# immunogenomics/harmony

Hardware: AMD Instinct MI355X
Metric: cells_per_sec_to_convergence (higher is better)
Workload: dtype f32

## Files before the change

### harmony_amd/csrc/hmx_api_diag.inc

```
int hmx_debug_seq_oe(const float* R, int64_t n, int32_t K, const int32_t* level, int32_t B, const int32_t* list, int64_t nlist,
                     const int32_t* chain_off, const int32_t* chain_cnt, int32_t nchains, int32_t seg_cells, int32_t passes, float* totals,
                     int64_t* mismatch, double* residual) {
  if (!R || !list || !level || !chain_off || !chain_cnt || !totals || n <= 0 || K <= 0 || B <= 0 || nchains <= 0 || seg_cells <= 0 || passes < 2) return HMX_ERR_ARG;
  if (nlist <= 0 || n > 2000000000ll || nlist > 2000000000ll || (size_t)B * 256 > 60 * 1024) return HMX_ERR_ARG;
  for (int64_t i = 0; i < nlist; i++) if (list[i] < 0 || list[i] >= n) return HMX_ERR_ARG;
  for (int64_t i = 0; i < n; i++) if (level[i] < 0 || level[i] >= B) return HMX_ERR_ARG;
  for (int c = 0; c < nchains; c++) if (chain_off[c] < 0 || chain_cnt[c] < 0 || (int64_t)chain_off[c] + chain_cnt[c] > nlist) return HMX_ERR_ARG;
  hmx_ctx* ctx = hmx_create();
  float* dR = nullptr; int* dl = nullptr; int* dlev = nullptr; int* dq = nullptr;
  auto run = [&]() -> int {
    int ndev = 0;
    if (hipGetDeviceCount(&ndev) != hipSuccess || ndev <= 0) return fail(ctx, HMX_ERR_DEVICE, "no HIP device");
    HIPCHK(hipStreamCreateWithFlags(&ctx->L.stream, hipStreamNonBlocking)); ctx->own_stream = true;
    HIPCHK(hipMalloc((void**)&dR, sizeof(float) * (size_t)n * K)); HIPCHK(hipMalloc((void**)&dl, sizeof(int) * (size_t)nlist));
    HIPCHK(hipMalloc((void**)&dlev, sizeof(int) * (size_t)n)); HIPCHK(hipMalloc((void**)&dq, sizeof(int) * (size_t)B));
    std::vector<int> ident(B); std::iota(ident.begin(), ident.end(), 0);
    CHK(h2d(ctx, dR, R, (size_t)n * K)); CHK(h2d(ctx, dl, list, (size_t)nlist)); CHK(h2d(ctx, dlev, level, (size_t)n)); CHK(h2d(ctx, dq, ident.data(), (size_t)B));
    ctx->K = K; ctx->B = B; ctx->seq_passes = passes; ctx->seq_stats = true;
    ctx->D.R = dR; ctx->D.K = K; ctx->D.B = B; ctx->D.C = 1; ctx->D.combo = dlev; ctx->D.qlev = dq;
    for (int c = 0; c < 4; c++) ctx->D.cov_end[c] = B;
    std::vector<std::pair<int, int>> ch;
    for (int c = 0; c < nchains; c++) ch.push_back({chain_off[c], chain_cnt[c]});
    CHK(seq_plan_build(ctx, ctx->plan_round, ch, seg_cells));
    CHK(seq_run_oe(ctx, ctx->plan_round, dl, nullptr, 0, nchains));
// ... 128 lines not shown
    if (ctx->L.stream && hipStreamSynchronize(ctx->L.stream) != hipSuccess) return -1;
    if (ctx->side && hipStreamSynchronize(ctx->side) != hipSuccess) return -1;
    return scalar(1.0);
  }
  if (f == "chain") return scalar((ctx->chain_ok || ctx->D.chain_pair) ? 1.0 : 0.0);
  if (f == "chain_wgs") return scalar((double)ctx->chain_wgs);
  if (f == "chain_pair") return scalar(ctx->D.chain_pair ? 1.0 : 0.0);
  if (f == "dot_bf") return scalar(ctx->D.dot_bf ? 1.0 : 0.0);
  if (f == "sold_carry") return scalar(ctx->carry_ok ? 1.0 : 0.0);
  if (f == "carried_rounds") return scalar((double)ctx->carried_rounds);
  if (f == "rounds_without_R") return scalar((double)ctx->rounds_without_R);
  if (f == "chain_rounds") return scalar((double)ctx->chain_rounds);
  if (f == "shuffle_inv") return scalar(ctx->shuf_inv ? 1.0 : 0.0);
  if (f == "p2p:exchange_us") return scalar(ctx->p2p_exchange_us);
  if (f == "p2p:allreduce_calls") return scalar((double)ctx->p2p_ar_calls);
  if (f == "p2p:allreduce_big_windows") return scalar((double)ctx->p2p_ar_big_windows);
  if (f == "p2p") return scalar(ctx->p2p_on && ctx->p2p_world == ctx->world ? 1.0 : 0.0);
  if (f == "chain_dbg") {
    if (!ctx->ran_setup) return -1;
    if (!out) return 64;
    std::vector<unsigned long long> h(64);
    if (d2h(ctx, h.data(), ctx->D.chain_dbg, 64)) return -1;
    (void)hipMemsetAsync(ctx->D.chain_dbg, 0, sizeof(unsigned long long) * 64, ctx->L.stream);
    return vec(h);
  }
  if (f.rfind("gputimer:", 0) == 0) {
    resolve_phases(ctx);
    const std::string nm = f.substr(9);
    if (nm == "Rcells_update") return hmx_get(ctx, "prof:update_ms", out, cap);
    auto it = ctx->gpu_timers.find(nm); return scalar(it == ctx->gpu_timers.end() ? 0.0 : it->second);
  }
  if (f.rfind("timer:", 0) == 0) { auto it = ctx->timers.find(f.substr(6)); return scalar(it == ctx->timers.end() ? 0.0 : it->second); }
  if (f == "seed_cells") return vec(ctx->seed_cells);
  if (f == "Y") return vec(ctx->Y);
  if (f == "W") return vec(ctx->W);
  if (f == "Pr_b") return vec(ctx->Pr_b);
  if (f == "theta") return vec(ctx->theta);
  if (f == "sigma") return vec(ctx->sigma);
  if (f == "lambda") return vec(ctx->lambda);
  if (f == "B_vec") return vec(ctx->B_vec);
  if (f == "objective_kmeans") return vec(ctx->obj_kmeans);
  if (f == "objective_kmeans_dist") return vec(ctx->obj_dist);
  if (f == "objective_kmeans_entropy") return vec(ctx->obj_entropy);
  if (f == "objective_kmeans_cross") return vec(ctx->obj_cross);
  if (f == "objective_harmony") return vec(ctx->obj_harmony);
  if (f == "kmeans_rounds") return vec(ctx->kmeans_rounds);
  if (ctx->query_done && (f == "Z_corr" || f == "Z_orig" || f == "R")) return hmx_get_matrix(ctx, field, out, HMX_F64, HMX_HOST, cap);
  if (!ctx->ran_setup) return -1;
  if (hipSetDevice(ctx->device) != hipSuccess) return -1;
  if (f == "ref_Nr" || f == "ref_C") {
    if (ctx->ran_init && !ctx->R_valid) { ctx->err = "R is not available: the clustering call that would have stored it did not complete"; return -1; }
    if (sync_solve_results(ctx)) return -1;
    const int K = ctx->K, d = ctx->d;
    const int64_t cnt = f == "ref_Nr" ? K : (int64_t)K * d;
    if (!out) return cnt;
    std::vector<double> res;
    if (ref_summary(ctx, res)) return -1;
    std::vector<double> v((size_t)cnt);
    for (int k = 0; k < K; k++) {
      if (f == "ref_Nr") v[k] = res[(size_t)k * (d + 1) + d];
      else for (int j = 0; j < d; j++) v[k + (size_t)K * j] = res[(size_t)k * (d + 1) + j];
    }
    return vec(v);
  }
  if (f == "seq:mismatch" || f == "seq:residual") {
    if (!ctx->sq_mismatch) return scalar(0.0);
// ... 133 lines not shown
```

### harmony_amd/csrc/hmx_api_kmeans.inc

```
int gather_centres(hmx_ctx* ctx, const std::vector<long long>& gcells, long long* d_gcells, double* d_rows) {
  const int K = ctx->K, d = ctx->d;
  CHK(h2d(ctx, d_gcells, gcells.data(), (size_t)K));
  l_gather_rows(ctx->L, ctx->D, d_gcells, (uint64_t)ctx->goff, d_rows); KCHK();
  CHK(allreduce(ctx, d_rows, (int64_t)K * d, 1));
  l_y_images(ctx->L, ctx->D, d_rows, 0); KCHK();
  ctx->y_on_device = true;
  return 0;
}

int kmeans_centers(hmx_ctx* ctx) {
  const int K = ctx->K, d = ctx->d;
  const Dev& D = ctx->D;
  ctx->Y.assign((size_t)d * K, 0.f);
  long long* const d_gcells = D.km_gcells; double* const d_rows = D.km_rows; unsigned* const d_excl = D.km_excl;
  std::vector<long long> gcells(K);
  const float Nm1 = (float)((uint64_t)ctx->N_global - 1);
  const bool rmode = ctx->rng_mode == 1;
  if (rmode) ensure_rrng(ctx);
  for (int i = 0; i < K; i++) gcells[i] = (long long)std::floor((rmode ? ctx->rrng.arma_randu() : hmx_u01(ctx->seed, 0, (uint64_t)i)) * Nm1);
  CHK(gather_centres(ctx, gcells, d_gcells, d_rows));
  std::vector<unsigned long long> win(K), sentinel(K, SEED_SENTINEL);
  std::set<unsigned> sup;
  if (rmode) {
    const int64_t n = ctx->N;
// ... 37 lines not shown
  } else {
  CHK(h2d(ctx, D.seedmin, sentinel.data(), (size_t)K));
  auto seed_probe = [&](const unsigned* excl, int nexcl) -> int {
    ctx->D.seed_key = ctx->seed; ctx->D.seed_goff = (unsigned long long)ctx->goff; ctx->D.seed_excl = excl; ctx->D.seed_nexcl = nexcl;
    l_tile_static(ctx->L, ctx->D, 3); KCHK();
    return 0;
  };
  CHK(seed_probe(nullptr, 0));
  CHK(allreduce(ctx, D.seedmin, K, 2));
  CHK(d2h(ctx, win.data(), D.seedmin, (size_t)K));
  for (int i = 0; i < K; i++) {
    unsigned g = (unsigned)(win[i] & 0xffffffffu);
    if (win[i] == SEED_SENTINEL) return fail(ctx, HMX_ERR_STATE, "centroid seeding found no candidate cell");
    if (sup.count(g)) {
      std::vector<unsigned> ex(sup.begin(), sup.end());
      CHK(h2d(ctx, d_excl, ex.data(), ex.size()));
      CHK(h2d(ctx, D.seedmin, sentinel.data(), (size_t)K));
      CHK(seed_probe(d_excl, (int)ex.size()));
      CHK(allreduce(ctx, D.seedmin, K, 2));
      std::vector<unsigned long long> w2(K);
      CHK(d2h(ctx, w2.data(), D.seedmin, (size_t)K));
      if (w2[i] == SEED_SENTINEL) return fail(ctx, HMX_ERR_STATE, "centroid seeding ran out of distinct cells");
      g = (unsigned)(w2[i] & 0xffffffffu);
    }
    sup.insert(g);
    gcells[i] = (long long)g;
  }
  }
  ctx->seed_cells.assign(gcells.begin(), gcells.end());
  CHK(gather_centres(ctx, gcells, d_gcells, d_rows));
  const bool tile_ok = (size_t)D.NQ * D.NS * 1024 + ((size_t)K * d + K) * 8 <= 160 * 1024;
  for (int it = 0; it < 10; it++) {
    if (it == 0) HIPCHK(hipMemsetAsync(D.lsum, 0, sizeof(long long) * ((size_t)K * d + K), ctx->L.stream));
    if (tile_ok) { l_tile_static(ctx->L, D, 2); KCHK(); }
    else { l_lloyd(ctx->L, D); KCHK(); }
    CHK(allreduce(ctx, D.lsum, (int64_t)K * d + K, 0));
    l_lloyd_finish(ctx->L, D); KCHK();
  }
  ctx->y_on_device = true;
  return 0;
}

void apply_set(Dev& D, const hmx_ctx::SortSet& s) {
  D.blk = s.blk; D.lorder = s.lorder; D.lpair = s.lpair; D.lcombo = s.lcombo; D.boff = s.boff; D.binoff = s.binoff; D.counts = s.counts; D.offs = s.offs; D.blkv = s.blkv; D.bincnt = s.bincnt;
}
int sort_group(hmx_ctx* ctx, uint64_t first) {
  const int nr = 4 - (int)(first & 3);
  SortBatch Sb{};
  Dev Dt = ctx->D; Dt.nxt = ctx->carry_ok ? 1 : 0;
  if (ctx->shuf_inv) {
    ShufSets T{};
    for (int r = 0; r < nr; r++) {
      const int os = (int)((first + (uint64_t)r) & 3);
      const hmx_ctx::SortSet& t = ctx->sets[os];
      T.posr[r] = ctx->posr[os]; T.lpair[r] = t.lpair; T.lorder[r] = t.lorder; T.lcombo[r] = t.lcombo; T.boff[r] = t.boff; T.partcnt[r] = ctx->shuf_partcnt[os]; T.binbase[r] = t.binoff; T.bincnt[r] = t.bincnt; T.binacc[r] = ctx->shuf_binacc[os];
    }
    l_shuffle_inv(ctx->L, Dt, T, nr, ctx->seed, first, (uint64_t)ctx->N_global, (uint64_t)ctx->goff, ctx->cells_per_block); KCHK();
  } else {
  for (int r = 0; r < nr; r++) {
    const hmx_ctx::SortSet& t = ctx->sets[(first + (uint64_t)r) & 3];
    Sb.p[r] = SortPtrs{t.blk, t.blkv, t.counts, t.offs, t.binoff, t.bincnt, t.boff, t.lorder, t.lcombo, t.lpair};
  }
  l_sort_batch(ctx->L, Dt, Sb, nr, ctx->seed, first, (uint64_t)ctx->N_global, (uint64_t)ctx->goff, ctx->cells_per_block); KCHK();
  }
  for (int r = 0; r < nr; r++) {
    const int os = (int)((first + (uint64_t)r) & 3);
    ctx->sorted_round[os] = (int64_t)first + r; ctx->sorted_seed[os] = ctx->seed; ctx->sorted_nxt[os] = Dt.nxt != 0; ctx->sorted_on_side[os] = false;
  }
  return 0;
}
int prepare_round(hmx_ctx* ctx, uint64_t round) {
  Dev& D = ctx->D;
  const int sset = (int)(round & (uint64_t)ctx->oset_mask);
// ... 56 lines not shown
```

### harmony_amd/csrc/hmx_api_p2p.inc

```
int hmx_p2p_export(hmx_ctx* ctx, uint8_t* handle_out) {
  if (!ctx || !handle_out) return ctx ? fail(ctx, HMX_ERR_ARG, "null handle buffer") : HMX_ERR_ARG;
  static_assert(sizeof(hipIpcMemHandle_t) == HMX_P2P_HANDLE_BYTES, "HIP IPC handle size");
  if (ctx->device < 0) { int cur = 0; (void)hipGetDevice(&cur); ctx->device = cur; }
  HIPCHK(hipSetDevice(ctx->device));
  if (!ctx->p2p_self) {
    const char* m = getenv("HMX_P2P_MEM");
    const unsigned flags = (m && std::string(m) == "uncached") ? hipDeviceMallocUncached : hipDeviceMallocFinegrained;
    void* p = nullptr;
    HIPCHK(hipExtMallocWithFlags(&p, P2P_INBOX_GRANULES * sizeof(unsigned long long), flags));
    HIPCHK(hipMemset(p, 0, P2P_INBOX_GRANULES * sizeof(unsigned long long)));
    HIPCHK(hipDeviceSynchronize());
    ctx->p2p_self = (unsigned long long*)p;
  }
  hipIpcMemHandle_t h;
  HIPCHK(hipIpcGetMemHandle(&h, ctx->p2p_self));
  std::memcpy(handle_out, &h, sizeof(h));
  return 0;
}
int hmx_p2p_connect(hmx_ctx* ctx, int32_t rank, int32_t world, const uint8_t* handles) {
  if (!ctx || !handles) return ctx ? fail(ctx, HMX_ERR_ARG, "null handle table") : HMX_ERR_ARG;
  if (world < 2 || world > 8 || rank < 0 || rank >= world) return fail(ctx, HMX_ERR_ARG, "the peer-to-peer chain takes 2..8 ranks");
  if (!ctx->p2p_self) return fail(ctx, HMX_ERR_STATE, "hmx_p2p_export first");
  HIPCHK(hipSetDevice(ctx->device));
  for (int g = 0; g < world; g++) {
// ... 104 lines not shown
  }
  ctx->injected.emplace_back(order, order + ctx->N_global);
  return 0;
}

int hmx_set_int(hmx_ctx* ctx, const char* field, int64_t v) {
  if (!ctx || !field) return HMX_ERR_ARG;
  const std::string f(field);
  if (f == "max_iter_kmeans") ctx->max_iter_kmeans = (int)v;
  else if (f == "seed") { ctx->seed = (uint64_t)v; ctx->rrng_seeded = false; }
  else if (f == "rng") { if (v != 0 && v != 1) return fail(ctx, HMX_ERR_ARG, "rng: 0 (counter-based) or 1 (R-compatible)"); ctx->rng_mode = (int)v; ctx->rrng_seeded = false; }
  else if (f == "ridge_arith" || f == "oe_arith" || f == "obj_arith" || f == "solve_arith" || f == "ref_arith") {
    if (v != 0 && v != 1 && !(f == "ref_arith" && v == 2)) return fail(ctx, HMX_ERR_ARG, f + ": 0 (exact accumulators) or 1 (the reference's fp32 operation order); ref_arith: also 2 (all groups but the O / E tables)");
    if (ctx->ran_setup) return fail(ctx, HMX_ERR_STATE, f + " must be set before setup");
    if (f == "ridge_arith" || f == "ref_arith") ctx->ridge_arith = v ? 1 : 0;
    if (f == "oe_arith" || f == "ref_arith") ctx->oe_arith = (v == 1) ? 1 : 0;
    if (f == "obj_arith" || f == "ref_arith") ctx->obj_arith = v ? 1 : 0;
    if (f == "solve_arith" || f == "ref_arith") ctx->solve_arith = v ? 1 : 0;
  }
  else if (f == "stale_dist") { if (ctx->ran_setup) return fail(ctx, HMX_ERR_STATE, "stale_dist must be set before setup"); ctx->stale_dist = v != 0; }
  else if (f == "seq_passes") { if (v < 2 || v > 64) return fail(ctx, HMX_ERR_ARG, "seq_passes: 2..64"); ctx->seq_passes = (int)v; if (ctx->seq_max_passes < (int)v) ctx->seq_max_passes = (int)v; }
  else if (f == "seq_warm_passes") { if (v < 1 || v > 64) return fail(ctx, HMX_ERR_ARG, "seq_warm_passes: 1..64"); ctx->seq_warm_passes = (int)v; }
  else if (f == "seq_stats") ctx->seq_stats = v != 0;
  else if (f == "seq_fused") { ctx->obj_fused = (int)(v & 1); ctx->ridge_kl = (int)((v >> 2) & 1); ctx->obj_dist_cache = (int)((v >> 3) & 1); }
  else if (f == "seq_tol_ppb") { if (v < 0 || v > 100000000) return fail(ctx, HMX_ERR_ARG, "seq_tol_ppb: 0 .. 1e8 (parts per billion)"); ctx->seq_tol = 1e-9 * (double)v; }
  else if (f == "seq_strict") { ctx->seq_strict = v != 0; if (v && ctx->seq_max_passes < 64) ctx->seq_max_passes = 64; }
  else if (f == "seq_max_passes") { if (v < 2 || v > 256) return fail(ctx, HMX_ERR_ARG, "seq_max_passes: 2..256"); ctx->seq_max_passes = (int)v; }
  else if (f == "device") ctx->device = (int)v;
  else if (f == "profile") { ctx->profile = (int)(v < 0 ? 0 : v > 2 ? 2 : v); ctx->prof_update_ms = 0; ctx->prof_update_launches = 0; ctx->prof_update_cells = 0; ctx->prof_update_steps = 0; ctx->ev_used = 0;
                             ctx->ph_used = 0; ctx->gpu_timers.clear(); }
  else if (f == "grid") { if (ctx->ran_setup) return fail(ctx, HMX_ERR_STATE, "grid must be set before setup"); ctx->L.grid = (int)v; }
  else if (f == "comm_force") ctx->comm_force = v != 0;
  else if (f == "upd_wps") { if (ctx->ran_setup) return fail(ctx, HMX_ERR_STATE, "upd_wps must be set before setup"); ctx->tun_wps = (int)v; }
  else if (f == "upd_debug") { if (ctx->ran_setup) ctx->D.upd_debug = (int)v; }
  else if (f == "upd_tpw") { ctx->tun_tpw = (int)v; if (ctx->ran_setup) ctx->D.upd_tpw = (int)(v < 1 ? 1 : v); }
  else return fail(ctx, HMX_ERR_ARG, "unknown or read-only field: " + f);
  return 0;
}
```

### harmony_amd/csrc/hmx_api_seam.inc

```
struct XferPool {
  std::vector<std::thread> th;
  const char* src = nullptr; char* dst = nullptr; size_t bytes = 0;
  std::atomic<size_t> next{0};
  std::atomic<int> gen{0}, running{0};
  std::atomic<bool> stop{false};
  static constexpr size_t CHUNK = 1 << 20;
  void work() {
    for (;;) {
      const size_t off = next.fetch_add(CHUNK);
      if (off >= bytes) break;
      memcpy(dst + off, src + off, std::min(CHUNK, bytes - off));
    }
  }
  void loop() {
    int seen = 0;
    for (;;) {
      int g;
      while ((g = gen.load(std::memory_order_acquire)) == seen) {
        if (stop.load(std::memory_order_relaxed)) return;
        __builtin_ia32_pause();
      }
      seen = g;
      work();
      running.fetch_sub(1, std::memory_order_release);
// ... 61 lines not shown
  const char* e = getenv("HMX_XFER_THREADS");
  const int t = e ? atoi(e) : 8, spare = (int)std::thread::hardware_concurrency() - 1;
  return std::max(0, std::min(std::min(t, 64), std::max(spare, 0)));
}

}

struct hmx_ctx {
  int rank = 0, world = 1;
  int64_t goff = 0, N_global = 0;
  hmx_allreduce_fn ar = nullptr; void* ar_user = nullptr;
  ncclComm_t comm = nullptr;
  int64_t comm_calls = 0, comm_bytes = 0;
  bool comm_force = false;
  unsigned long long* p2p_self = nullptr; unsigned long long* p2p_peer[8] = {}; int p2p_rank = 0, p2p_world = 0; bool p2p_on = false;
  unsigned p2p_tests = 0; int* p2p_result = nullptr; double p2p_exchange_us = 0.0; std::string p2p_note = "not connected";
  unsigned p2p_ar_seq = 0, p2p_xseq = 0; int64_t p2p_ar_calls = 0, p2p_ar_big_windows = 0;
  int (*poll)(void*) = nullptr; void* poll_user = nullptr;
  int64_t N = 0;
  int d = 0, K = 0, B = 0, C = 0, Q = 0;
  std::vector<int> B_vec, cov_bounds;
  std::vector<float> sigma, theta, lambda, Pr_b, sizes;
  bool lambda_estimation = false;
  float alpha = 0.2f, block_size = 0.05f, eps_k = 1e-3f, eps_h = 1e-2f, cutoff = 1e-5f;
  int max_iter_kmeans = 4, window_size = 3, verbose = 0;
  uint64_t seed = 0, round_counter = 0;
  int nb = 20; uint64_t cells_per_block = 1;
  std::vector<float> Y;
  std::vector<float> W; int W_rows = 0;
  std::vector<float> obj_kmeans, obj_dist, obj_entropy, obj_cross, obj_harmony;
  std::vector<int> kmeans_rounds;
  std::vector<int> qlev, perm;
  std::vector<long long> seed_cells;
  std::deque<std::vector<int64_t>> injected;
  int64_t subset_clusters = 0, skipped_clusters = 0;
  double* h_obj = nullptr; int obj_cap = 0, obj_pending = 0; hipEvent_t obj_event = nullptr; bool obj_harmony_pending = false;
  int rng_mode = 0; hmx::RRng rrng; bool rrng_seeded = false;
  bool solve_on_device = true, y_on_device = false, solve_pending = false;
  double* sv_cov = nullptr; double* sv_rhs = nullptr; float* sv_Wall = nullptr; int* sv_mrows = nullptr; int* sv_flags = nullptr;
  float* sv_lambda = nullptr; int* sv_cov_bounds = nullptr;
  int ridge_arith = 0, oe_arith = 0, obj_arith = 0, solve_arith = 0;
  int stale_dist = 0; float* Zc_head = nullptr; float* Yt_head = nullptr; bool head_is_stale = false;
  struct SeqPlan { SeqSeg* d_segs = nullptr; SeqChain* d_chains = nullptr; size_t cap_segs = 0, cap_chains = 0; int nsegs = 0, nchains = 0;
                   std::vector<int> seg0;    int seg_cells = 0; std::vector<int> cells;    };
  SeqPlan plan_head, plan_ridge, plan_round, plan_pair;
  int* pairlist = nullptr; int* pair_idx = nullptr; int npairs = 0;
  float* rg_tot = nullptr; float* rp_tot = nullptr; float* rp_start = nullptr; bool rp_warm = false;
  float* sq_start = nullptr; float* sq_end = nullptr; size_t sq_cap = 0;
  float* sq_total = nullptr; size_t sq_total_cap = 0;
  unsigned* sq_mismatch = nullptr; int seq_passes = 2, seq_warm_passes = 2; int64_t seq_runs = 0;
  bool seq_scan_final = false;
  bool seq_stats = false;
  unsigned* sq_conv = nullptr; int seq_max_passes = 24; int64_t seq_adaptive_cells = 200000, seq_extra_passes = 0; double seq_resid_max = 0.0; uint64_t seq_mismatch_sum = 0;
  double seq_tol = 1e-5;
  bool seq_strict = false; uint64_t seq_last_mismatch = 0, seq_unsettled = 0; double seq_oe_cell_passes = 0.0;
  int64_t seq_group_passes[4] = {0, 0, 0, 0}, seq_group_runs[4] = {0, 0, 0, 0};
  int* headlist = nullptr;
  int* headq = nullptr;
  std::vector<int> lev_off, lev_cnt;
  int* headlev = nullptr; int* roundlev = nullptr;
  int* roundlist = nullptr;
  std::vector<int> invperm_h, combo_h;
  float* Of = nullptr; float* Ef = nullptr; float* Mtab = nullptr;
  float* objT = nullptr; size_t objT_cap = 0;
  float* objD = nullptr; size_t objD_cap = 0; bool objD_valid = false, in_cluster_rounds = false;
  struct ObjfRun { Launch L; Dev D; int mat = 0; long long nt = 0; const float* T = nullptr; float* tot = nullptr; double* objv = nullptr; int np = 0, done = 0; bool adaptive = false; };
// ... 318 lines not shown
```

### harmony_amd/csrc/hmx_internal.h

```cpp
#pragma once
#include <hip/hip_runtime.h>
#include <stdint.h>

namespace hmx {

constexpr int WAVE = 64;
constexpr int TPB = 256;
constexpr int ITEM_CELLS = 256;
constexpr int APPLY_CELLS = 1024;
constexpr int SORT_CHUNK = 512;
constexpr float FX_SCALE = 536870912.0f;
constexpr double FX_INV = 1.0 / 536870912.0;

struct Item { int q; int start; int cnt; };

struct Dev {
  int n;
  int d, K, B, C, Q;
  int B0;
  int cov_end[4];
  int dot_bf;
  int KP;
  int zs;
  int NCT;
// ... 133 lines not shown
  hipEvent_t ev0 = nullptr, ev1 = nullptr;
};

void l_convert_in(const Launch& L, const void* src, int f32, float* dst, const int* invperm, int n, int d, int zs);
void l_convert_out(const Launch& L, const float* src, void* dst, int f32, const int* invperm, int n, int w, int ws);
void l_copy(const Launch& L, const float* src, float* dst, size_t count);
void l_zero4(const Launch& L, void* a, size_t na, void* b, size_t nb, void* c, size_t nc, void* d, size_t nd);
void l_normalize(const Launch& L, float* Z, int n, int d, int zs);
void l_normalize_from(const Launch& L, const float* src, float* dst, int n, int d, int zs);
void l_head(const Launch& L, const Dev& D);
void l_tile_static(const Launch& L, const Dev& D, int mode);
void l_sort_blocks(const Launch& L, const Dev& D, bool fused, uint64_t seed, uint64_t round, uint64_t Nglob, uint64_t goff,
                   uint64_t cells_per_block);
void l_sort_hist(const Launch& L, const Dev& D, bool fused, uint64_t seed, uint64_t round, uint64_t Nglob, uint64_t goff, uint64_t cells_per_block);
void l_sort_tail(const Launch& L, const Dev& D);
struct SortPtrs { int* blk; int* blkv; int* counts; int* offs; int* binoff; int* bincnt; int* boff; int* lorder; int* lcombo; int2* lpair; };
struct SortBatch { SortPtrs p[4]; };
struct ShufSets { int2* posr[4]; int2* lpair[4]; int* lorder[4]; int* lcombo[4]; int* boff[4]; int* partcnt[4]; int* binbase[4]; int* bincnt[4]; int* binacc[4]; };
int shuffle_parts(uint64_t Nglob, int nb, uint64_t cells_per_block);
void l_shuffle_blocks(const Launch& L, const Dev& D, uint64_t seed, uint64_t round, uint64_t Nglob, uint64_t goff, uint64_t cells_per_block);
void l_shuffle_inv(const Launch& L, const Dev& D, const ShufSets& T, int nr, uint64_t seed, uint64_t round, uint64_t Nglob, uint64_t goff,
                   uint64_t cells_per_block);
void l_sort_batch(const Launch& L, const Dev& D, const SortBatch& S, int nr, uint64_t seed, uint64_t round, uint64_t Nglob, uint64_t goff,
                  uint64_t cells_per_block);
void l_oldsum(const Launch& L, const Dev& D);
void l_fold(const Launch& L, const Dev& D, int j, int mode);
void l_penalty(const Launch& L, const Dev& D);
void l_foldpen(const Launch& L, const Dev& D, int j, const long long* Oin, long long* Oout, const long long* Sin,
               long long* Szero);
void l_obj_reduce(const Launch& L, const Dev& D);
void l_update(const Launch& L, const Dev& D, int j);
void l_chain(const Launch& L, const Dev& D, int workgroups);
void l_tile_static_bf(const Launch& L, const Dev& D, int mode);
void l_update_bf(const Launch& L, const Dev& D, int j);
void l_chain_bf(const Launch& L, const Dev& D, int workgroups);
void l_round_tail(const Launch& L, const Dev& D, double* host_slot, long long* z0, size_t n0, long long* z1, size_t n1);
__host__ __device__ constexpr int kcol(int nct, int ct, int c) {
  return ct < 4 * (nct >> 2) ? 64 * (ct >> 2) + 4 * c + (ct & 3) : 64 * (nct >> 2) + (nct & 3) * c + (ct - 4 * (nct >> 2));
}
__host__ __device__ inline void kcol_inv(int nct, int k, int& qd, int& i, int& c) {
  const int nfull = nct >> 2, r = nct & 3;
  if (k < 64 * nfull) { qd = k >> 6; c = (k & 63) >> 2; i = k & 3; }
  else { qd = nfull; const int kk = k - 64 * nfull; c = kk / r; i = kk - c * r; }
}
__host__ __device__ inline void bf3_split(float x, unsigned short (&p)[3]) {
  union { float f; unsigned u; } a, b;
  a.f = x;
  p[0] = (unsigned short)(a.u >> 16);
  b.u = a.u & 0xffff0000u;
  a.f = x - b.f;
  p[1] = (unsigned short)(a.u >> 16);
  b.u = a.u & 0xffff0000u;
  a.f = a.f - b.f;
  p[2] = (unsigned short)(a.u >> 16);
}
__host__ __device__ inline size_t bfimg_index(int nct, int ns2, int j, int k, int part) {
  int qd, i, c;
  kcol_inv(nct, k, qd, i, c);
  const int ct = 4 * qd + i, s = j >> 5, g = (j & 31) >> 3;
  return ((((size_t)ct * ns2 + s) * 3 + part) * 64 + 16 * g + c) * 8 + (j & 7);
}
__host__ __device__ inline void bfimg_store(unsigned short* img, int nct, int ns2, int j, int k, float y) {
  unsigned short p[3];
  bf3_split(y, p);
  for (int part = 0; part < 3; part++) img[bfimg_index(nct, ns2, j, k, part)] = p[part];
}
__host__ __device__ inline void bfimg_store_all(const Dev& D, int j, int k, float y) {
  bfimg_store(D.Yimg3, D.NCT, D.NS2, j, k, y);
  if (D.Yimg3p) {
    const int nctp = (D.KH + 15) >> 4, h = k >= D.KH ? 1 : 0;
    bfimg_store(D.Yimg3p + (size_t)h * nctp * D.NS2 * 3 * 512, nctp, D.NS2, j, h ? k - D.KH : k, y);
  }
}
constexpr int P2P_CAP = 65536;
constexpr int P2P_PLANES = 4;
constexpr size_t P2P_TEST_BASE = (size_t)P2P_PLANES * 8 * P2P_CAP * 2;
constexpr size_t P2P_INBOX_GRANULES = P2P_TEST_BASE + 64;
void l_p2p_allreduce(const Launch& L, const Dev& D, void* buf, int n, int dtype, unsigned seq, int* err);
void l_p2p_allreduce_big(const Launch& L, const Dev& D, void* buf, int n, int dtype, unsigned seq, int* err);
void l_p2p_selftest(const Launch& L, const Dev& D, unsigned tag, int* result);
void l_objective_tables(const Launch& L, const Dev& D);
void l_moe_stats(const Launch& L, const Dev& D);
void l_moe_apply(const Launch& L, const Dev& D);
void l_moe_stats_mfma(const Launch& L, const Dev& D);
void l_moe_solve(const Launch& L, const Dev& D, const SolveArgs& A);
void l_moe_apply_mfma(const Launch& L, const Dev& D);
void l_seed_race_u(const Launch& L, const Dev& D, const float* u, int a0, int na, int only, uint64_t goff, const unsigned* excl,
                   int nexcl);
void l_gather_rows(const Launch& L, const Dev& D, const long long* gcells, uint64_t goff, double* rows);
void l_lloyd(const Launch& L, const Dev& D);
void l_lloyd_finish(const Launch& L, const Dev& D);
void l_y_images(const Launch& L, const Dev& D, const double* rows, int normalise);
size_t lds_bytes_y(const Dev& D);

struct QueryDev {
  int n, d, K, zs, KP16;
  const float* Z;
  const float* yhat;
  const float* sig2;
  const Item* chunks; int nchunks;
  int slice;
  double* part;
  const float* Zsum; const float* Rsum;
  const float* Wq; int w_lds;
  float* out; float* Rout;
};
constexpr int QUERY_SLICE = 6144;
void l_query_stats(const Launch& L, const QueryDev& Q, int summary);
void l_query_fold(const Launch& L, const double* part, const int* qchunk, int nq, int total, double* out);
void l_query_apply(const Launch& L, const QueryDev& Q);

struct SeqSeg { int off; int cnt; };
struct SeqChain { int seg0; int nseg; };
void l_seq_oe_pass(const Launch& L, const Dev& D, const int* list, const int* poslev, int nlist, const SeqSeg* segs, int seg0, int nsegs, const float* start,
                   float* end, int zero_start, unsigned* conv_zero);
void l_seq_sum_pass(const Launch& L, const Dev& D, const int* list, const SeqSeg* segs, int seg0, int nsegs, const float* start, float* end,
                    int zero_start, unsigned* conv_zero);
void l_ref_posord(const Launch& L, const Dev& D, uint64_t seed, uint64_t round, uint64_t Nglob, int* posord, int* poslev);
void l_seq_ridge_pass(const Launch& L, const Dev& D, const int* list, const int* listq, const SeqSeg* segs, int seg0, int nsegs, const unsigned char* inset,
                      const float* start, float* end, int zero_start, unsigned* conv_zero);
bool l_seq_ridge_pass_kl(const Launch& L, const Dev& D, const int* list, const SeqSeg* segs, int seg0, int nsegs, const unsigned char* inset,
                         const float* start, float* end, int zero_start, unsigned* conv_zero);
// ... 22 lines not shown
```

### harmony_amd/csrc/hmx_k_launch.inc

```
#if HMX_TILE_BF
#define HMX_LNAME(x) x##_bf
#else
#define HMX_LNAME(x) x
size_t lds_bytes_y(const Dev& D) { return (size_t)D.d * D.KP * sizeof(float); }
#endif
static inline size_t bf_image_bytes(const Dev& D) { return (size_t)D.NCT * D.NS2 * 3 * 1024; }
static inline size_t tile_image_bytes(const Dev& D) { return HMX_TILE_BF ? bf_image_bytes(D) : (size_t)D.NQ * D.NS * 64 * sizeof(f32x4); }
constexpr size_t LDS_PER_CU = 160 * 1024;
static inline bool bf_fits(const Dev& D, size_t rest, long long blocks) {
  const long long per_cu = (blocks + 255) / 256;
  return D.dot_bf && D.Yimg3 && (bf_image_bytes(D) + rest) * (size_t)(per_cu < 1 ? 1 : per_cu) <= LDS_PER_CU;
}

#if !HMX_TILE_BF
#define HMX_DISPATCH_KD(KERNEL, GRID, LDS, ...)                                                \
  do {                                                                                         \
    const int kpl_ = D.KP / 64, dpl_ = D.d > 64 ? 2 : 1;                                       \
    if (dpl_ == 1) {                                                                           \
      switch (kpl_) {                                                                          \
        case 1: hipLaunchKernelGGL((KERNEL<1, 1>), GRID, dim3(TPB), LDS, L.stream, __VA_ARGS__); break; \
        case 2: hipLaunchKernelGGL((KERNEL<2, 1>), GRID, dim3(TPB), LDS, L.stream, __VA_ARGS__); break; \
        case 3: hipLaunchKernelGGL((KERNEL<3, 1>), GRID, dim3(TPB), LDS, L.stream, __VA_ARGS__); break; \
        default: hipLaunchKernelGGL((KERNEL<4, 1>), GRID, dim3(TPB), LDS, L.stream, __VA_ARGS__); break; \
      }                                                                                        \
// ... 60 lines not shown
#endif
  const size_t lds = tile_image_bytes(D) + rest;
  const dim3 grid((unsigned)blocks);
#if HMX_TILE_BF
  if (mode == 2 && thr == 512 && D.NCT >= 5 && D.NCT <= 7) {
    switch (D.NCT) {
      case 5: hipLaunchKernelGGL((k_tile<5, 2, 3>), grid, dim3(768), lds, L.stream, D, 0); break;
      case 6: hipLaunchKernelGGL((k_tile<6, 2, 3>), grid, dim3(768), lds, L.stream, D, 0); break;
      default: hipLaunchKernelGGL((k_tile<7, 2, 3>), grid, dim3(768), lds, L.stream, D, 0); break;
    }
    return;
  }
#endif
#define HMX_TS(N) case N: if (mode == 3) hipLaunchKernelGGL((k_tile<N, 3>), grid, dim3(thr), lds, L.stream, D, 0); \
                          else if (mode == 2) hipLaunchKernelGGL((k_tile<N, 2>), grid, dim3(thr), lds, L.stream, D, 0); \
                          else if (D.usig) hipLaunchKernelGGL((k_tile<N, 1, 2, true>), grid, dim3(thr), lds, L.stream, D, 0); \
                          else hipLaunchKernelGGL((k_tile<N, 1>), grid, dim3(thr), lds, L.stream, D, 0); break;
#define HMX_TSL(N) case N: hipLaunchKernelGGL((k_tile<N, 1, 4, true>), grid, dim3(thr), lds, L.stream, D, 0); break;
  if (mode == 1 && D.upd_wps == 4) {
    switch (D.NCT) {
      HMX_TSL(1) HMX_TSL(2) HMX_TSL(3) HMX_TSL(4)
      default: break;
    }
    return;
  }
  switch (D.NCT) {
    HMX_TS(1) HMX_TS(2) HMX_TS(3) HMX_TS(4) HMX_TS(5) HMX_TS(6) HMX_TS(7) HMX_TS(8)
    HMX_TS(10) HMX_TS(12) HMX_TS(13) HMX_TS(14) HMX_TS(16)
    default: break;
  }
#undef HMX_TS
#undef HMX_TSL
}
#if !HMX_TILE_BF
void l_head(const Launch& L, const Dev& D) {
  HMX_DISPATCH_KD(k_head, dim3(stream_grid(L, D.nitems)), lds_bytes_y(D), D);
}
static SortPtrs sort_ptrs_of(const Dev& D) { return SortPtrs{D.blk, D.blkv, D.counts, D.offs, D.binoff, D.bincnt, D.boff, D.lorder, D.lcombo, D.lpair}; }
static BlockIdArgs block_id_args(uint64_t seed, uint64_t round, uint64_t Nglob, uint64_t goff, uint64_t cells_per_block) {
  BlockIdArgs A;
  A.fk = make_keys(seed, round, Nglob); A.fk2 = make_keys(seed, round + 1, Nglob); A.Nglob = Nglob; A.goff = goff; A.cpb = cells_per_block;
  A.inv_cpb = 1.0f / (float)cells_per_block;
  return A;
}
void l_sort_hist(const Launch& L, const Dev& D, bool fused, uint64_t seed, uint64_t round, uint64_t Nglob, uint64_t goff, uint64_t cells_per_block) {
  const int nV = D.nxt ? D.nb * D.nb : D.nb;
  const size_t lds = (size_t)nV * sizeof(int);
  BlockIdBatch AB{}; AB.a[0] = block_id_args(seed, round, Nglob, goff, cells_per_block);
  SortBatch S{}; S.p[0] = sort_ptrs_of(D);
  if (fused) hipLaunchKernelGGL(k_sort_hist<true>, dim3(D.nchunks), dim3(WAVE), lds, L.stream, D, AB, S);
  else hipLaunchKernelGGL(k_sort_hist<false>, dim3(D.nchunks), dim3(WAVE), lds, L.stream, D, AB, S);
}
void l_sort_tail(const Launch& L, const Dev& D) {
  const int nV = D.nxt ? D.nb * D.nb : D.nb;
  const size_t lds = (size_t)nV * sizeof(int);
  SortBatch S{}; S.p[0] = sort_ptrs_of(D);
  hipLaunchKernelGGL(k_sort_binscan, dim3(nV * D.Q), dim3(WAVE), 0, L.stream, D, S);
  hipLaunchKernelGGL(k_sort_binoff, dim3(1), dim3(1024), 0, L.stream, D, S);
  hipLaunchKernelGGL(k_sort_scatter, dim3(D.nchunks), dim3(WAVE), lds, L.stream, D, S);
}
void l_sort_blocks(const Launch& L, const Dev& D, bool fused, uint64_t seed, uint64_t round, uint64_t Nglob, uint64_t goff,
                   uint64_t cells_per_block) {
  l_sort_hist(L, D, fused, seed, round, Nglob, goff, cells_per_block);
  l_sort_tail(L, D);
}
void l_sort_batch(const Launch& L, const Dev& D, const SortBatch& S, int nr, uint64_t seed, uint64_t round, uint64_t Nglob, uint64_t goff,
// ... 529 lines not shown
```

### harmony_amd/csrc/hmx_k_tile.inc

```

__device__ __forceinline__ float dpp_f(float v, const int ctrl_id) {
  const int x = __float_as_int(v);
  int r;
  switch (ctrl_id) {
    case 0: r = __builtin_amdgcn_update_dpp(0, x, 0xB1, 0xF, 0xF, true); break;
    case 1: r = __builtin_amdgcn_update_dpp(0, x, 0x4E, 0xF, 0xF, true); break;
    case 2: r = __builtin_amdgcn_update_dpp(0, x, 0x141, 0xF, 0xF, true); break;
    default: r = __builtin_amdgcn_update_dpp(0, x, 0x140, 0xF, 0xF, true); break;
  }
  return __int_as_float(r);
}
__device__ __forceinline__ float rowsum16(float v) {
  v += dpp_f(v, 0);
  v += dpp_f(v, 1);
  v += dpp_f(v, 2);
  v += dpp_f(v, 3);
  return v;
}

template <int NF>
__global__ __launch_bounds__(TPB) void k_normalize4(const float* Zsrc, float* Z, int n, int nq) {
  const int lane = threadIdx.x & 63, c = lane & 15, g = lane >> 4;
  const int wave = (blockIdx.x * blockDim.x + threadIdx.x) >> 6, nw = (gridDim.x * blockDim.x) >> 6;
  const f32x4 zero4 = {0.f, 0.f, 0.f, 0.f};
// ... 1595 lines not shown
      f32x4 acc[NCT];
      dots_stream(D.Zc + (size_t)(cellA.x >= 0 ? cellA.x : 0) * zs, cellA.x >= 0, acc);
      epilogue(cellA.x, tile_q(cellA), acc);
    }
  }
  if constexpr (MODE == 2) {
    __syncthreads();
    for (int i = threadIdx.x; i < K * D.d; i += blockDim.x)
      if (ltab[i]) atomicAdd((unsigned long long*)&D.lsum[i], (unsigned long long)ltab[i]);
    for (int i = threadIdx.x; i < K; i += blockDim.x)
      if (ltab[K * D.d + i]) atomicAdd(&D.lcnt[i], (unsigned long long)ltab[K * D.d + i]);
  } else if constexpr (MODE == 3) {
#pragma unroll
    for (int ct = 0; ct < NCT; ct++) {
      unsigned long long v = best[ct];
      unsigned long long o = shfl_xor_u64(v, 16); v = o < v ? o : v;
      o = shfl_xor_u64(v, 32); v = o < v ? o : v;
      if (g == 0 && kcol(NCT, ct, c) < K && v != ~0ull) atomicMin(&D.seedmin[kcol(NCT, ct, c)], v);
    }
  } else {
    if (ts >= te) return;
    if (curq >= 0) flush_run();
    od = wsumd(od); oe = wsumd(oe);
    if (lane == 0) {
      const int slotrow = (MODE == 0) ? (j % D.objslots) : 0;
      double* slot = D.objpart + ((size_t)slotrow * D.nwmax + wave) * 2;
      if (MODE == 0 && D.nb <= D.objslots) { slot[0] = od; slot[1] = oe; }
      else { slot[0] += od; slot[1] += oe; }
    }
    stamp(6);
    stamp(7);
  }
}
```

Measured before the change: 76.76 million.

## Add dedicated LDS-tiled Lloyd k-means kernel with block-local fixed-point accumulation

Adds a k_lloyd_tile kernel used in the k-means initialisation loop when the centre image and the per-block sum table fit in LDS. It computes distances with tile dot products, picks the nearest centre per cell through DPP reductions, and accumulates fixed-point sums and counts in LDS before flushing to global atomics. The intent is to cut the global atomic traffic and generic tile-kernel overhead of the previous l_tile_static path. It also adds a probe API for comparing the two implementations. Risks include LDS pressure limiting occupancy, and the change only affects the fixed ten Lloyd iterations.

```diff
diff --git a/harmony_amd/csrc/hmx_api_diag.inc b/harmony_amd/csrc/hmx_api_diag.inc
--- a/harmony_amd/csrc/hmx_api_diag.inc
+++ b/harmony_amd/csrc/hmx_api_diag.inc
@@ -184,6 +184,8 @@
   }
   if (f.rfind("timer:", 0) == 0) { auto it = ctx->timers.find(f.substr(6)); return scalar(it == ctx->timers.end() ? 0.0 : it->second); }
   if (f == "seed_cells") return vec(ctx->seed_cells);
+  if (f == "lloyd_probe:sums") return vec(ctx->lloyd_probe_sums);
+  if (f == "lloyd_probe:centres") return vec(ctx->lloyd_probe_centres);
   if (f == "Y") return vec(ctx->Y);
   if (f == "W") return vec(ctx->W);
   if (f == "Pr_b") return vec(ctx->Pr_b);
diff --git a/harmony_amd/csrc/hmx_api_kmeans.inc b/harmony_amd/csrc/hmx_api_kmeans.inc
--- a/harmony_amd/csrc/hmx_api_kmeans.inc
+++ b/harmony_amd/csrc/hmx_api_kmeans.inc
@@ -93,13 +93,44 @@
   const bool tile_ok = (size_t)D.NQ * D.NS * 1024 + ((size_t)K * d + K) * 8 <= 160 * 1024;
   for (int it = 0; it < 10; it++) {
     if (it == 0) HIPCHK(hipMemsetAsync(D.lsum, 0, sizeof(long long) * ((size_t)K * d + K), ctx->L.stream));
-    if (tile_ok) { l_tile_static(ctx->L, D, 2); KCHK(); }
+    if (tile_ok) { if (!l_lloyd_tile(ctx->L, D)) l_tile_static(ctx->L, D, 2); KCHK(); }
     else { l_lloyd(ctx->L, D); KCHK(); }
     CHK(allreduce(ctx, D.lsum, (int64_t)K * d + K, 0));
     l_lloyd_finish(ctx->L, D); KCHK();
   }
   ctx->y_on_device = true;
   return 0;
+}
+
+int lloyd_probe(hmx_ctx* ctx, int impl) {
+  const int K = ctx->K, d = ctx->d;
+  const Dev& D = ctx->D;
+  if (!ctx->ran_setup || !ctx->y_on_device) return fail(ctx, HMX_ERR_STATE, "lloyd_probe: needs centres on the device (kmeans_centers first)");
+  if (ctx->world > 1) return fail(ctx, HMX_ERR_STATE, "lloyd_probe: one rank only");
+  const size_t nt = (size_t)K * d + K;
+  float* keep = nullptr;
+  HIPCHK(hipMalloc((void**)&keep, sizeof(float) * (size_t)K * d));
+  int st = 0;
+  auto step = [&]() -> int {
+    HIPCHK(hipMemcpyAsync(keep, D.Ycur, sizeof(float) * (size_t)K * d, hipMemcpyDeviceToDevice, ctx->L.stream));
+    HIPCHK(hipMemsetAsync(D.lsum, 0, sizeof(long long) * nt, ctx->L.stream));
+    const bool tile_ok = (size_t)D.NQ * D.NS * 1024 + nt * 8 <= 160 * 1024;
+    if (!tile_ok) l_lloyd(ctx->L, D);
+    else if (impl == 0 || !l_lloyd_tile(ctx->L, D)) l_tile_static(ctx->L, D, 2);
+    KCHK();
+    ctx->lloyd_probe_sums.resize(nt);
+    CHK(d2h(ctx, ctx->lloyd_probe_sums.data(), (const long long*)D.lsum, nt));
+    l_lloyd_finish(ctx->L, D); KCHK();
+    ctx->lloyd_probe_centres.resize((size_t)K * d);
+    CHK(d2h(ctx, ctx->lloyd_probe_centres.data(), (const float*)D.Ycur, (size_t)K * d));
+    HIPCHK(hipMemcpyAsync(D.Ycur, keep, sizeof(float) * (size_t)K * d, hipMemcpyDeviceToDevice, ctx->L.stream));
+    l_y_images(ctx->L, D, nullptr, 0); KCHK();
+    HIPCHK(hipStreamSynchronize(ctx->L.stream));
+    return 0;
+  };
+  st = step();
+  (void)hipFree(keep);
+  return st;
 }
 
 void apply_set(Dev& D, const hmx_ctx::SortSet& s) {
diff --git a/harmony_amd/csrc/hmx_api_p2p.inc b/harmony_amd/csrc/hmx_api_p2p.inc
--- a/harmony_amd/csrc/hmx_api_p2p.inc
+++ b/harmony_amd/csrc/hmx_api_p2p.inc
@@ -160,6 +160,7 @@
   else if (f == "grid") { if (ctx->ran_setup) return fail(ctx, HMX_ERR_STATE, "grid must be set before setup"); ctx->L.grid = (int)v; }
   else if (f == "comm_force") ctx->comm_force = v != 0;
   else if (f == "upd_wps") { if (ctx->ran_setup) return fail(ctx, HMX_ERR_STATE, "upd_wps must be set before setup"); ctx->tun_wps = (int)v; }
+  else if (f == "lloyd_probe") return lloyd_probe(ctx, (int)v);
   else if (f == "upd_debug") { if (ctx->ran_setup) ctx->D.upd_debug = (int)v; }
   else if (f == "upd_tpw") { ctx->tun_tpw = (int)v; if (ctx->ran_setup) ctx->D.upd_tpw = (int)(v < 1 ? 1 : v); }
   else return fail(ctx, HMX_ERR_ARG, "unknown or read-only field: " + f);
diff --git a/harmony_amd/csrc/hmx_api_seam.inc b/harmony_amd/csrc/hmx_api_seam.inc
--- a/harmony_amd/csrc/hmx_api_seam.inc
+++ b/harmony_amd/csrc/hmx_api_seam.inc
@@ -117,6 +117,7 @@
   std::vector<int> kmeans_rounds;
   std::vector<int> qlev, perm;
   std::vector<long long> seed_cells;
+  std::vector<long long> lloyd_probe_sums; std::vector<float> lloyd_probe_centres;
   std::deque<std::vector<int64_t>> injected;
   int64_t subset_clusters = 0, skipped_clusters = 0;
   double* h_obj = nullptr; int obj_cap = 0, obj_pending = 0; hipEvent_t obj_event = nullptr; bool obj_harmony_pending = false;
diff --git a/harmony_amd/csrc/hmx_internal.h b/harmony_amd/csrc/hmx_internal.h
--- a/harmony_amd/csrc/hmx_internal.h
+++ b/harmony_amd/csrc/hmx_internal.h
@@ -189,6 +189,7 @@
 void l_update(const Launch& L, const Dev& D, int j);
 void l_chain(const Launch& L, const Dev& D, int workgroups);
 void l_tile_static_bf(const Launch& L, const Dev& D, int mode);
+bool l_lloyd_tile_bf(const Launch& L, const Dev& D);
 void l_update_bf(const Launch& L, const Dev& D, int j);
 void l_chain_bf(const Launch& L, const Dev& D, int workgroups);
 void l_round_tail(const Launch& L, const Dev& D, double* host_slot, long long* z0, size_t n0, long long* z1, size_t n1);
@@ -245,6 +246,7 @@
 void l_seed_race_u(const Launch& L, const Dev& D, const float* u, int a0, int na, int only, uint64_t goff, const unsigned* excl,
                    int nexcl);
 void l_gather_rows(const Launch& L, const Dev& D, const long long* gcells, uint64_t goff, double* rows);
+bool l_lloyd_tile(const Launch& L, const Dev& D);
 void l_lloyd(const Launch& L, const Dev& D);
 void l_lloyd_finish(const Launch& L, const Dev& D);
 void l_y_images(const Launch& L, const Dev& D, const double* rows, int normalise);
diff --git a/harmony_amd/csrc/hmx_k_launch.inc b/harmony_amd/csrc/hmx_k_launch.inc
--- a/harmony_amd/csrc/hmx_k_launch.inc
+++ b/harmony_amd/csrc/hmx_k_launch.inc
@@ -116,6 +116,29 @@
 #undef HMX_TS
 #undef HMX_TSL
 }
+bool HMX_LNAME(l_lloyd_tile)(const Launch& L, const Dev& D) {
+  if (D.NT4 > 4 || D.NCT > 8) return false;
+  const size_t rest = ((size_t)D.K * D.d + D.K) * sizeof(long long);
+#if !HMX_TILE_BF
+  if (bf_fits(D, rest, 256)) return l_lloyd_tile_bf(L, D);
+#else
+  if (D.NS2 > 2) return false;
+#endif
+  const size_t lds = tile_image_bytes(D) + rest;
+  if (lds > LDS_PER_CU) return false;
+  constexpr int WPS = 2, wpb = 4 * WPS;
+  long long blocks = ((long long)D.ntitems + 2 * wpb - 1) / (2 * wpb);
+  if (blocks > 256) blocks = 256;
+  if (blocks < 1) blocks = 1;
+  const dim3 grid((unsigned)blocks);
+#define HMX_LT(N) case N: hipLaunchKernelGGL((k_lloyd_tile<N, WPS>), grid, dim3(256 * WPS), lds, L.stream, D); break;
+  switch (D.NCT) {
+    HMX_LT(1) HMX_LT(2) HMX_LT(3) HMX_LT(4) HMX_LT(5) HMX_LT(6) HMX_LT(7) HMX_LT(8)
+    default: return false;
+  }
+#undef HMX_LT
+  return true;
+}
 #if !HMX_TILE_BF
 void l_head(const Launch& L, const Dev& D) {
   HMX_DISPATCH_KD(k_head, dim3(stream_grid(L, D.nitems)), lds_bytes_y(D), D);
diff --git a/harmony_amd/csrc/hmx_k_tile.inc b/harmony_amd/csrc/hmx_k_tile.inc
--- a/harmony_amd/csrc/hmx_k_tile.inc
+++ b/harmony_amd/csrc/hmx_k_tile.inc
@@ -1651,3 +1651,154 @@
     stamp(7);
   }
 }
+
+
+
+template <int NCT, int WPS, bool BF = (HMX_TILE_BF != 0)>
+__global__ __launch_bounds__(256 * WPS) void k_lloyd_tile(Dev D) {
+  extern __shared__ __attribute__((aligned(16))) f32x4 lds4[];
+  const int K = D.K, zs = D.zs, dd = D.d;
+  const int nY4 = BF ? NCT * D.NS2 * 3 * 64 : D.NQ * D.NS * 64;
+  const u32x4* const ldsB = reinterpret_cast<const u32x4*>(lds4);
+  long long* const ltab = reinterpret_cast<long long*>(lds4 + nY4);
+  const int lane = threadIdx.x & 63, c = lane & 15, g = lane >> 4;
+  const int nw = (int)((gridDim.x * blockDim.x) >> 6);
+  const int wave = __builtin_amdgcn_readfirstlane((int)((blockIdx.x * blockDim.x + threadIdx.x) >> 6));
+  const int ntiles = D.ntitems, per = 2 * ((ntiles + 2 * nw - 1) / (2 * nw));
+  const int ts = min(ntiles, wave * per), te = min(ntiles, ts + per);
+  const int rowmask = BF ? rows_mask_bf(g, zs) : 0;
+  auto ld_rows = [&](const float* __restrict__ zr, RowRegs& r) __attribute__((always_inline)) {
+    if constexpr (BF) load_rows_bf(zr, g, zs, r); else load_rows(zr, g, D.NT4, D.tail, r);
+  };
+  auto tile_cell = [&](int tile) -> int {
+    if (tile >= te) return -1;
+    const Item* tp = D.titems + tile;
+    asm volatile("" : "+v"(tp));
+    const Item it = *tp;
+    return (c < it.cnt) ? it.start + c : -1;
+  };
+  auto row_of = [&](const int cell) { return D.Zc + (size_t)(cell >= 0 ? cell : 0) * zs; };
+  int cellA = tile_cell(ts), cellB = tile_cell(ts + 1);
+  RowRegs rowsA, rowsB;
+  {
+    const int bd = blockDim.x, tid = threadIdx.x;
+    const f32x4* src = BF ? reinterpret_cast<const f32x4*>(D.Yimg3) : reinterpret_cast<const f32x4*>(D.Yimg);
+    {
+      f32x4 t[4];
+#pragma unroll
+      for (int k = 0; k < 4; k++) t[k] = src[min(tid + k * bd, nY4 - 1)];
+#pragma unroll
+      for (int k = 0; k < 4; k++) if (tid + k * bd < nY4) lds4[tid + k * bd] = t[k];
+    }
+    ld_rows(row_of(cellA), rowsA);
+    ld_rows(row_of(cellB), rowsB);
+    for (int base = 4 * bd; base < nY4; base += 4 * bd) {
+      f32x4 t[4];
+#pragma unroll
+      for (int k = 0; k < 4; k++) t[k] = src[min(base + tid + k * bd, nY4 - 1)];
+#pragma unroll
+      for (int k = 0; k < 4; k++) if (base + tid + k * bd < nY4) lds4[base + tid + k * bd] = t[k];
+    }
+    for (int i = tid; i < K * dd + K; i += bd) ltab[i] = 0;
+    __syncthreads();
+  }
+  float yn[NCT];
+#pragma unroll
+  for (int ct = 0; ct < NCT; ct++) {
+    const bool kv = kcol(NCT, ct, c) < K;
+    yn[ct] = ld_or(D.ynorm, (size_t)min(kcol(NCT, ct, c), K - 1), kv, 0.0f);
+  }
+  auto epilogue = [&](const int cell, const RowRegs& rows, const f32x4 (&acc)[NCT]) __attribute__((always_inline)) {
+    float bs[4]; int bk[4];
+#pragma unroll
+    for (int reg = 0; reg < 4; reg++) {
+      bs[reg] = INFINITY; bk[reg] = 0x7fffffff;
+#pragma unroll
+      for (int ct = 0; ct < NCT; ct++) {
+        const float sc = (ct < first_partial_ct(NCT) || kcol(NCT, ct, c) < K) ? fmaf(acc[ct][reg], -2.0f, yn[ct]) : INFINITY;
+        const bool lt = sc < bs[reg];
+        bs[reg] = lt ? sc : bs[reg];
+        bk[reg] = lt ? kcol(NCT, ct, c) : bk[reg];
+      }
+    }
+    float m[4];
+#pragma unroll
+    for (int reg = 0; reg < 4; reg++) m[reg] = bs[reg];
+#pragma unroll
+    for (int st = 0; st < 4; st++) {
+      float t[4];
+#pragma unroll
+      for (int reg = 0; reg < 4; reg++) t[reg] = (st == 0) ? dpp_f(m[reg], 0) : (st == 1) ? dpp_f(m[reg], 1) : (st == 2) ? dpp_f(m[reg], 2) : dpp_f(m[reg], 3);
+#pragma unroll
+      for (int reg = 0; reg < 4; reg++) m[reg] = fminf(m[reg], t[reg]);
+    }
+    int kb[4];
+#pragma unroll
+    for (int reg = 0; reg < 4; reg++) kb[reg] = (bs[reg] == m[reg]) ? bk[reg] : 0x7fffffff;
+#pragma unroll
+    for (int st = 0; st < 4; st++) {
+      int t[4];
+#pragma unroll
+      for (int reg = 0; reg < 4; reg++) {
+        const float kf = __int_as_float(kb[reg]);
+        t[reg] = __float_as_int((st == 0) ? dpp_f(kf, 0) : (st == 1) ? dpp_f(kf, 1) : (st == 2) ? dpp_f(kf, 2) : dpp_f(kf, 3));
+      }
+#pragma unroll
+      for (int reg = 0; reg < 4; reg++) kb[reg] = min(kb[reg], t[reg]);
+    }
+    int t4[4];
+#pragma unroll
+    for (int reg = 0; reg < 4; reg++) t4[reg] = __shfl(kb[reg], 16 * (c >> 2), 64);
+    const int kc = min(((c & 3) == 0) ? t4[0] : ((c & 3) == 1) ? t4[1] : ((c & 3) == 2) ? t4[2] : t4[3], K - 1);
+    if (cell >= 0) {
+      long long* row = ltab + (size_t)kc * dd;
+      if constexpr (BF) {
+#pragma unroll
+        for (int t = 0; t < 4; t++) {
+#pragma unroll
+          for (int e = 0; e < 4; e++) {
+            const int jj = 32 * (t >> 1) + 8 * g + 4 * (t & 1) + e;
+            if (t < 2 * D.NS2 && jj < dd) atomicAdd((unsigned long long*)&row[jj], (unsigned long long)(long long)__float2int_rn(rows.v[t][e] * 1073741824.0f));
+          }
+        }
+      } else {
+#pragma unroll
+        for (int t = 0; t < 4; t++) {
+          if (t < D.NT4) {
+#pragma unroll
+            for (int e = 0; e < 4; e++) {
+              const int jj = 16 * t + 4 * g + e;
+              if (jj < dd) atomicAdd((unsigned long long*)&row[jj], (unsigned long long)(long long)__float2int_rn(rows.v[t][e] * 1073741824.0f));
+            }
+          }
+        }
+#pragma unroll
+        for (int u = 0; u < 3; u++) {
+          const int jj = 16 * D.NT4 + 4 * u + g;
+          if (u < D.tail && jj < dd) atomicAdd((unsigned long long*)&row[jj], (unsigned long long)(long long)__float2int_rn(rows.t[u] * 1073741824.0f));
+        }
+      }
+      if (g == 0) atomicAdd((unsigned long long*)&ltab[K * dd + kc], 1ull);
+    }
+  };
+  for (int tile = ts; tile < te; tile += 2) {
+    const int cellC = cellA, cellD = cellB;
+    const RowRegs rowsC = rowsA, rowsD = rowsB;
+    cellA = tile_cell(tile + 2); cellB = tile_cell(tile + 3);
+    ld_rows(row_of(cellA >= 0 ? cellA : cellC), rowsA);
+    ld_rows(row_of(cellB >= 0 ? cellB : cellD), rowsB);
+    f32x4 accC[NCT], accD[NCT];
+    if constexpr (BF) tile_dots_bf_regs2<NCT>(ldsB, rowsC, cellC >= 0, rowsD, cellD >= 0, rowmask, lane, D.NS2, accC, accD);
+    else {
+      tile_dots_regs<NCT>(lds4, rowsC, cellC >= 0, lane, D.NS, D.NT4, D.tail, accC);
+      tile_dots_regs<NCT>(lds4, rowsD, cellD >= 0, lane, D.NS, D.NT4, D.tail, accD);
+    }
+    epilogue(cellC, rowsC, accC);
+    epilogue(cellD, rowsD, accD);
+  }
+  __syncthreads();
+  for (int i = threadIdx.x; i < K * dd; i += blockDim.x)
+    if (ltab[i]) atomicAdd((unsigned long long*)&D.lsum[i], (unsigned long long)ltab[i]);
+  for (int i = threadIdx.x; i < K; i += blockDim.x)
+    if (ltab[K * dd + i]) atomicAdd(&D.lcnt[i], (unsigned long long)ltab[K * dd + i]);
+}
```

After: 76.77 million, median of 3. About the same (+0.0%).
